# Siyou-Li/u2Tokenizer

Measured on AMD Instinct MI355X. Metric: CT volumes/sec (256^3 fp16) through u2Tokenizer fwd, higher is better.
Workload: dtype bf16; 1 GPU; BASELINE configs[2]: u2Qwen3-8B-shaped path, 256^3 volume = 8x(32,256,256) fp16, ViT-B 3D x12, SPP, 4-layer rma+diffts+dmtp tokenizer (8 heads, top_k 1024, scales {1,2,4}, 256 queries), text 1024, prompt 1024; hidden_size=4096, batch_per_gpu=1, streams_per_gpu=2, parallelism=replicas x1, tta_side_stream=off in the multi-stream run, on in the one-stream run

## Files before the change

include/u2tok.h:

```cpp
#ifndef U2TOK_H_
#define U2TOK_H_

#include <stddef.h>
#include <stdint.h>

#ifdef __cplusplus
extern "C" {
#endif

#define U2TOK_OK 0
#define U2TOK_ERR_ARG (-1)
#define U2TOK_ERR_LAUNCH (-2)
#define U2TOK_ERR_WORKSPACE (-3)
#define U2TOK_ERR_DEVICE (-4)

typedef void* u2tok_stream_t;

int u2tok_version(void);
const char* u2tok_arch(void);
const char* u2tok_elem(void);
int u2tok_device_check(void);
typedef struct u2tok_ctx* u2tok_ctx_t;
int u2tok_ctx_create(u2tok_ctx_t* out);
int u2tok_ctx_destroy(u2tok_ctx_t ctx);
// ... 67 lines not shown
int u2tok_tokenizer_forward(const u2tok_tokenizer_config* cfg, const void* const* weights, const void* v_token,
                            const void* t_token, void* out, int64_t* topk_idx_out, void* svr_out, void* workspace,
                            size_t workspace_bytes, u2tok_stream_t stream);

typedef struct {
  const void* const* svr_in;
  void* const* svr_out;
  const void* visual_in;
  void* visual_out;
  const void* const* tta_in;
  void* const* tta_out;
} u2tok_tokenizer_taps;
int u2tok_tokenizer_forward_taps(const u2tok_tokenizer_config* cfg, const void* const* weights, const void* v_token,
                                 const void* t_token, void* out, int64_t* topk_idx_out, const u2tok_tokenizer_taps* taps,
                                 void* workspace, size_t workspace_bytes, u2tok_stream_t stream);

int u2tok_embed_splice(const void* table, const int64_t* ids, const void* feats, void* out, int32_t B, int32_t S,
                       int32_t E, int32_t nfeat, int64_t vocab, u2tok_stream_t stream);

size_t u2tok_preprocess_workspace_bytes(int32_t D, int32_t H, int32_t W);
int u2tok_preprocess_volume(const float* vol, void* out, int32_t* info, int32_t D, int32_t H, int32_t W, int32_t target,
                            int32_t depth_pad, float lower_pct, float upper_pct, int32_t out_dtype, void* workspace,
                            size_t workspace_bytes, u2tok_stream_t stream);

typedef struct {
  int32_t rot90_k;
  int32_t flip[3];
  float scale_factor;
  float shift_offset;
} u2tok_augment;
// ... 158 lines not shown
```

u2tokenizer_amd/_lib.py:

```python
from __future__ import annotations

import ctypes as C
import os
import subprocess
import threading
from pathlib import Path

_PKG = Path(__file__).resolve().parent
_LIB = _PKG / "lib" / "libu2tok_hip.so"
_LIBS = {"bf16": _LIB, "f16": _PKG / "lib" / "libu2tok_hip_f16.so"}
_lock = threading.Lock()
_handles = {}


class LibraryNotBuilt(RuntimeError):
    pass


def lib_path() -> Path:
    return _LIB


def build(verbose: bool = False) -> Path:
    cmd = ["make", "-C", str(_PKG / "csrc"), "-j", str(os.cpu_count() or 4)]
# ... 55 lines not shown
    "u2tok_ctx_destroy": (_i32, [_vp]),
    "u2tok_ctx_set_current": (_i32, [_vp]),
    "u2tok_ctx_get_current": (_vp, []),
    "u2tok_set_option": (_i32, [C.c_char_p, _i32]),
    "u2tok_profile_collect": (_i32, [_vp, _vp, _vp, _i32]),
    "u2tok_profile_collect2": (_i32, [_vp, _vp, _vp, _vp, _i32]),
    "u2tok_set_gemm_scratch": (_i32, [_vp, _sz, _vp]),
    "u2tok_vit_workspace_bytes": (_sz, [C.POINTER(VitConfig)]),
    "u2tok_vit_forward": (_i32, [C.POINTER(VitConfig), C.POINTER(_vp), _vp, _vp, _vp, _sz, _vp]),
    "u2tok_spp_workspace_bytes": (_sz, [C.POINTER(SppConfig)]),
    "u2tok_spp_forward": (_i32, [C.POINTER(SppConfig), C.POINTER(_vp), _vp, _vp, _vp, _sz, _vp]),
    "u2tok_tokenizer_workspace_bytes": (_sz, [C.POINTER(TokConfig)]),
    "u2tok_tokenizer_forward": (_i32, [C.POINTER(TokConfig), C.POINTER(_vp), _vp, _vp, _vp, _vp, _vp, _vp, _sz, _vp]),
    "u2tok_tokenizer_forward_taps": (_i32, [C.POINTER(TokConfig), C.POINTER(_vp), _vp, _vp, _vp, _vp, C.POINTER(TokTaps),
                                            _vp, _sz, _vp]),
    "u2tok_tok_attention_workspace_bytes": (_sz, [_i32, _i32, _i32, _i32, _i32]),
    "u2tok_tok_attention": (_i32, [_vp, _vp, _vp, _vp, _i32, _i32, _i32, _i32, _i32, _i64, _i64, _i64, _i64, _i64, _i64, _i64,
                                   _i64, _f32, _vp, _i32, _i32, _vp, _sz, _vp]),
    "u2tok_preprocess_workspace_bytes": (_sz, [_i32, _i32, _i32]),
    "u2tok_preprocess_volume": (_i32, [_vp, _vp, _vp, _i32, _i32, _i32, _i32, _i32, _f32, _f32, _i32, _vp, _sz, _vp]),
    "u2tok_preprocess_volume_aug": (_i32, [_vp, _vp, _vp, _i32, _i32, _i32, _i32, _i32, _f32, _f32, _i32,
                                           C.POINTER(Augment), _vp, _sz, _vp]),
    "u2tok_embed_splice": (_i32, [_vp, _vp, _vp, _vp, _i32, _i32, _i32, _i32, _i64, _vp]),
    "u2tok_gemm_bf16": (_i32, [_vp, _vp, _vp, _vp, _vp, _i32, _i32, _i32, _i64, _i64, _i64, _i64, _i32, _i32,
                               _i64, _i64, _i64, _i64, _i64, _i64, _i64, _i64, _f32, _i32, _vp]),
    "u2tok_layernorm_bf16": (_i32, [_vp, _vp, _vp, _vp, _vp, _i32, _i32, _f32, _vp]),
    "u2tok_softmax_rows": (_i32, [_vp, _vp, _i32, _i32, _i32, _i64, _i64, _f32, _vp, _i32, _i32, _vp]),
    "u2tok_transpose_bf16": (_i32, [_vp, _vp, _i32, _i32, _i32, _i64, _i64, _i64, _i64, _i32, _vp]),
    "u2tok_im2col_patches": (_i32, [_vp, _i32, _vp, _i32, _i32, _i32, _i32, _i32, _i32, _i32, _vp]),
    "u2tok_avgpool3d_tokens": (_i32, [_vp, _vp, _i32, _i32, _i32, _i32, _i32, _i32, _i32, _i32, _vp]),
# ... 109 lines not shown
```

u2tokenizer_amd/csrc/capi.hip:

```cpp
#include <math.h>
#include <string.h>
#include <new>
#include "pipeline.h"

using namespace u2;

static_assert(U2TOK_OK == U2_OK && U2TOK_ERR_ARG == U2_ERR_ARG && U2TOK_ERR_LAUNCH == U2_ERR_LAUNCH &&
                  U2TOK_ERR_WORKSPACE == U2_ERR_WORKSPACE && U2TOK_ERR_DEVICE == U2_ERR_DEVICE,
              "public and internal status codes must agree");

#define BF(p) reinterpret_cast<const bf16_t*>(p)
#define BFW(p) reinterpret_cast<bf16_t*>(p)
#define ST(s) reinterpret_cast<hipStream_t>(s)

extern "C" {

int u2tok_version(void) { return 200;  }
const char* u2tok_arch(void) { return "gfx950"; }
const char* u2tok_elem(void) { return U2_ELEM_ASM; }

int u2tok_device_check(void) {
  int dev = 0;
  if (hipGetDevice(&dev) != hipSuccess) return U2_ERR_DEVICE;
  hipDeviceProp_t prop;
// ... 21 lines not shown

int u2tok_set_option(const char* name, int value) {
  if (!name) return U2_ERR_ARG;
  Options& o = ctx().opt;
  struct Opt { const char* name; int Options::*field; int lo, hi; };
  static const Opt table[] = {
      {"gemm_splitk", &Options::gemm_splitk, -1, 16},   {"gemm_mubuf", &Options::gemm_mubuf, 0, 1}, {"ln_wide", &Options::ln_wide, 0, 1},   {"gemm_big", &Options::gemm_big, -1, 27},
      {"gemm_big_grid", &Options::gemm_big_grid, 1, 4096}, {"gemm_big_splitk", &Options::gemm_big_splitk, 0, 16},
      {"gemm_big_drain", &Options::gemm_big_drain, 0, 1}, {"gemm_skinny", &Options::gemm_skinny, 0, 2},
       {"kmajor_b", &Options::kmajor_b, 0, 1},            {"gemm_tail_fused", &Options::gemm_tail_fused, 0, 1},
      {"flash_mode", &Options::flash_mode, 0, 7},        {"flash_q_prescaled", &Options::flash_q_prescaled, 0, 1},
      {"vit_flash", &Options::vit_flash, 0, 1},         {"tta_overlap", &Options::tta_overlap, 0, 1},
      {"vit_vt_epilogue", &Options::vit_vt_epilogue, 0, 1},
      {"tok_flash", &Options::tok_flash, 0, 1},
      {"tok_wide", &Options::tok_wide, 0, 2},
  };
  if (!strcmp(name, "gemm_tile")) {
    if (value != 0 && value != 64 && value != 128) return U2_ERR_ARG;
    o.gemm_tile = value;
    return U2_OK;
  }
  if (!strcmp(name, "profile")) { prof_enable(value != 0); return U2_OK; }
  for (const Opt& t : table)
    if (!strcmp(name, t.name)) {
      if (value < t.lo || value > t.hi) return U2_ERR_ARG;
      if (t.field == &Options::gemm_big && value > 0 && !(value >= 20 && value <= 27 && value != 23 && value != 25)) return U2_ERR_ARG;
      if (t.field == &Options::flash_mode && value != 0 && value != 1 && value != 7) return U2_ERR_ARG;
      o.*(t.field) = value;
      return U2_OK;
    }
// ... 29 lines not shown
size_t u2tok_spp_workspace_bytes(const u2tok_spp_config* cfg) {
  if (!cfg) return 0;
  size_t peak = 0;
  if (spp_forward(*cfg, nullptr, nullptr, nullptr, nullptr, 0, true, &peak, nullptr) != U2_OK) return 0;
  return peak + 256;
}
int u2tok_spp_forward(const u2tok_spp_config* cfg, const void* const* weights, const void* x, void* out,
                      void* workspace, size_t workspace_bytes, u2tok_stream_t stream) {
  if (!cfg || !workspace || ((uintptr_t)workspace & 255)) return U2_ERR_ARG;
  return spp_forward(*cfg, weights, BF(x), BFW(out), workspace, workspace_bytes, false, nullptr, ST(stream));
}

size_t u2tok_tokenizer_workspace_bytes(const u2tok_tokenizer_config* cfg) {
  if (!cfg) return 0;
  size_t peak = 0;
  if (tokenizer_forward(*cfg, nullptr, nullptr, nullptr, nullptr, nullptr, nullptr, nullptr, nullptr, 0, true, &peak,
                        nullptr) != U2_OK)
    return 0;
  return peak + 256;
}
int u2tok_tokenizer_forward(const u2tok_tokenizer_config* cfg, const void* const* weights, const void* v_token,
                            const void* t_token, void* out, int64_t* topk_idx_out, void* svr_out, void* workspace,
                            size_t workspace_bytes, u2tok_stream_t stream) {
  if (!cfg || !workspace || ((uintptr_t)workspace & 255)) return U2_ERR_ARG;
  return tokenizer_forward(*cfg, weights, BF(v_token), BF(t_token), BFW(out), topk_idx_out, BFW(svr_out), nullptr, workspace,
                           workspace_bytes, false, nullptr, ST(stream));
}
int u2tok_tokenizer_forward_taps(const u2tok_tokenizer_config* cfg, const void* const* weights, const void* v_token,
                                 const void* t_token, void* out, int64_t* topk_idx_out, const u2tok_tokenizer_taps* taps,
                                 void* workspace, size_t workspace_bytes, u2tok_stream_t stream) {
  if (!cfg || !taps || !workspace || ((uintptr_t)workspace & 255)) return U2_ERR_ARG;
  return tokenizer_forward(*cfg, weights, BF(v_token), BF(t_token), BFW(out), topk_idx_out, nullptr, taps, workspace,
                           workspace_bytes, false, nullptr, ST(stream));
}

size_t u2tok_preprocess_workspace_bytes(int32_t D, int32_t H, int32_t W) { return preprocess_workspace_bytes(D, H, W); }
int u2tok_preprocess_volume(const float* vol, void* out, int32_t* info, int32_t D, int32_t H, int32_t W, int32_t target,
                            int32_t depth_pad, float lower_pct, float upper_pct, int32_t out_dtype, void* workspace,
                            size_t workspace_bytes, u2tok_stream_t stream) {
  return preprocess_volume(vol, out, info, D, H, W, target, depth_pad, lower_pct, upper_pct, out_dtype, nullptr, workspace,
                           workspace_bytes, ST(stream));
}
int u2tok_preprocess_volume_aug(const float* vol, void* out, int32_t* info, int32_t D, int32_t H, int32_t W, int32_t target,
                                int32_t depth_pad, float lower_pct, float upper_pct, int32_t out_dtype,
                                const u2tok_augment* aug, void* workspace, size_t workspace_bytes, u2tok_stream_t stream) {
  if (!aug) return U2_ERR_ARG;
  PreAugment a;
  a.rot_k = aug->rot90_k;
// ... 324 lines not shown
```

u2tokenizer_amd/csrc/ctx.h:

```cpp
#pragma once
#include <mutex>
#include <vector>
#include "common.h"

namespace u2 {

struct Options {
  int ln_wide = 1;
  int gemm_tile = 0;
  int gemm_mubuf = 1;
  int gemm_splitk = 0;
  int gemm_big = 0;
  int gemm_big_grid = 256;
  int gemm_big_splitk = 0;
  int gemm_big_drain = 1;
  int gemm_skinny = 2;
  int gemm_tail_fused = 1;
  int kmajor_b = 1;
  int flash_mode = 0;
  int flash_q_prescaled = 0;
  int vit_flash = 1;
  int vit_vt_epilogue = 1;
  int tok_flash = 1;
  int tok_wide = 2;
  int tta_overlap = 1;
  int profile = 0;
};

struct SideStream {
  hipStream_t owner = nullptr;
  hipStream_t s = nullptr;
  hipEvent_t fork = nullptr;
  hipEvent_t done[16] = {};
};

struct Scratch {
  hipStream_t st;
  void* p;
  size_t bytes;
};
// ... 30 lines not shown
```

u2tokenizer_amd/csrc/pipeline.h:

```cpp
#pragma once
#include <algorithm>
#include "../../include/u2tok.h"
#include "kernels.h"

namespace u2 {

typedef u2tok_vit_config VitConfig;
typedef u2tok_spp_config SppConfig;
typedef u2tok_tokenizer_config TokConfig;
typedef u2tok_tokenizer_taps TokTaps;

int vit_forward(const VitConfig& c, const void* const* W, const void* volume, bf16_t* out, void* ws, size_t ws_bytes,
                bool dry, size_t* peak, hipStream_t st);
int spp_forward(const SppConfig& c, const void* const* W, const bf16_t* x, bf16_t* out, void* ws, size_t ws_bytes,
                bool dry, size_t* peak, hipStream_t st);
int tokenizer_forward(const TokConfig& c, const void* const* W, const bf16_t* v_token, const bf16_t* t_token,
                      bf16_t* out, int64_t* topk_idx_out, bf16_t* svr_out, const TokTaps* taps, void* ws, size_t ws_bytes,
                      bool dry, size_t* peak, hipStream_t st);

}
```

u2tokenizer_amd/csrc/pipeline.hip:

```cpp
#include "pipeline.h"

namespace u2 {

namespace {

struct Arena {
  char* base;
  size_t cap;
  size_t off = 0, peak = 0;
  bool dry;
  Arena(void* b, size_t c, bool d) : base((char*)b), cap(c), dry(d) {}
  template <typename T>
  T* get(size_t count) {
    const size_t a = (off + 255) & ~(size_t)255;
    off = a + count * sizeof(T);
    if (off > peak) peak = off;
    if (dry) return reinterpret_cast<T*>((uintptr_t)0x1000 + a);
    return (off <= cap) ? reinterpret_cast<T*>(base + a) : nullptr;
  }
  bool ok() const { return dry || peak <= cap; }
};

struct ScratchScope {
  Context& cx;
// ... 275 lines not shown
  return a.wk && a.bk && a.wv == a.wk + (size_t)E * E && a.bv == a.bk + E;
}
inline bool qkv_packed(const Att& a, int E) {
  return a.wq && a.bq && a.wk == a.wq + (size_t)E * E && a.bk == a.bq + E && kv_packed(a, E);
}
int qkv_proj(const bf16_t* x, const Att& a, bf16_t* out, int64_t rows, int E, bool dry, hipStream_t st) {
  if (!dry && qkv_packed(a, E)) {
    U2_RUN(linear(x, E, a.wq, a.bq, out, 3 * E, rows, E, 3 * E, 0, nullptr, 0, st));
    return U2_OK;
  }
  U2_RUN(linear(x, E, a.wq, a.bq, out, 3 * E, rows, E, E, 0, nullptr, 0, st));
  U2_RUN(linear(x, E, a.wk, a.bk, out + E, 3 * E, rows, E, E, 0, nullptr, 0, st));
  U2_RUN(linear(x, E, a.wv, a.bv, out + 2 * E, 3 * E, rows, E, E, 0, nullptr, 0, st));
  return U2_OK;
}
}

int tokenizer_forward(const TokConfig& c, const void* const* W, const bf16_t* v_token, const bf16_t* t_token,
                      bf16_t* out, int64_t* topk_idx_out, bf16_t* svr_out, const TokTaps* taps, void* ws, size_t ws_bytes,
                      bool dry, size_t* peak, hipStream_t st) {
  if (c.B <= 0 || c.T <= 0 || c.N <= 0 || c.E <= 0 || c.Lt <= 0 || c.num_heads <= 0 || c.num_layers < 0) return U2_ERR_ARG;
  if (c.E % c.num_heads || (c.E / c.num_heads) % 8 || c.top_k <= 0 || c.num_query <= 0) return U2_ERR_ARG;
  if (c.attn_type < 0 || c.attn_type > 2) return U2_ERR_ARG;
  if (!dry && (!W || !v_token || !t_token || !out)) return U2_ERR_ARG;
  const int B = c.B, T = c.T, N = c.N, E = c.E, H = c.num_heads, d = E / H, L = c.num_layers, Q = c.num_query;
  const int TN = T * N, k = c.top_k;
  if (!c.enable_diffts && k > TN) return U2_ERR_ARG;
  if (N > c.max_seq_len || T > c.max_seq_len || Q > c.max_seq_len) return U2_ERR_ARG;
  const float scale = 1.0f / sqrtf((float)d);
  auto wp = [&](int i) { return dry ? nullptr : reinterpret_cast<const bf16_t*>(W[i]); };
  auto att_at = [&](int i) {
    Att a{wp(i), wp(i + 1), wp(i + 2), wp(i + 3), wp(i + 4), wp(i + 5), wp(i + 6), wp(i + 7), wp(i + 8)};
    if (c.attn_type != 0) a.rb = nullptr;
    return a;
  };
  const int i_sel = 1 + 18 * L, i_gate = i_sel + 2, i_tta = i_gate + 2, i_lin = i_tta + 33 * L;

  Arena ar(ws, ws_bytes, dry);
  const size_t kSplitK = std::max<size_t>(24u << 20, (size_t)16 * B * c.num_query * 3 * E);
  char* skw = ar.get<char>(kSplitK);
  U2_CHECK_WS(ar);
  Context& cx = ctx();
  ScratchScope scratch_scope(cx, st, skw, kSplitK, !dry);
  const int64_t rows = (int64_t)B * TN;
  bf16_t* xa = ar.get<bf16_t>((size_t)rows * E);
  bf16_t* xb = ar.get<bf16_t>((size_t)rows * E);
  bf16_t* qkv = ar.get<bf16_t>((size_t)rows * 3 * E);
  bf16_t* ctx = ar.get<bf16_t>((size_t)rows * E);
  U2_CHECK_WS(ar);

  const bf16_t* x = v_token;
  for (int l = 0; l < L; ++l) {
    const Att sp = att_at(1 + 18 * l), tp = att_at(1 + 18 * l + 9);
    if (taps && !dry && taps->svr_in && taps->svr_in[l]) x = reinterpret_cast<const bf16_t*>(taps->svr_in[l]);
// ... 157 lines not shown
  if (overlap && !dry) {
    if (hipEventRecord(side->fork, st) != hipSuccess || hipStreamWaitEvent(side->s, side->fork, 0) != hipSuccess)
      return U2_ERR_LAUNCH;
    for (int l = 0; l < L; ++l) {
      const int base = i_tta + 33 * l;
      Att va = att_at(base + 9), ta = att_at(base + 18);
      { const int e = kv_proj(va, V, Lv, kv_v[l], side->s); if (e != U2_OK) return e; }
      if (hipEventRecord(side->done[2 * l], side->s) != hipSuccess) return U2_ERR_LAUNCH;
      { const int e = kv_proj(ta, t_token, c.Lt, kv_t[l], side->s); if (e != U2_OK) return e; }
      if (hipEventRecord(side->done[2 * l + 1], side->s) != hipSuccess) return U2_ERR_LAUNCH;
    }
    const Att la = att_at(i_lin);
    U2_RUN(linear(V, E, la.wk, la.bk, k_lin, E, (int64_t)B * Lv, E, E, 0, nullptr, 0, side->s));
    if (hipEventRecord(side->done[2 * L], side->s) != hipSuccess) return U2_ERR_LAUNCH;
  }
  U2_RUN(fill_rows(wp(0), qa, B, (int64_t)Q * E, (int64_t)Q * E, st));
  bf16_t* qcur = qa;
  auto cross = [&](const Att& a, const bf16_t* src, int Ls, const bf16_t* qin, bf16_t* dst, bf16_t* kv,
                   int kv_ready) -> int {
    U2_RUN(linear(qin, E, a.wq, a.bq, qproj, E, qrows, E, E, 0, nullptr, 0, st));
    if (kv_ready < 0) {
      const int e = kv_proj(a, src, Ls, kv, st);
      if (e != U2_OK) return e;
    } else if (!dry) {
      if (hipStreamWaitEvent(st, side->done[kv_ready], 0) != hipSuccess) return U2_ERR_LAUNCH;
    }
    AttnCore ac{qproj, kv, kv + E, E, 2 * E, 2 * E, (int64_t)Q * E, (int64_t)Ls * 2 * E, (int64_t)Ls * 2 * E,
                qctx, E, (int64_t)Q * E, B, Q, Ls, H, d, scale, nullptr, 0};
    const int e = attention_core(ar, ac, dry, st);
    if (e != U2_OK) return e;
    U2_RUN(linear(qctx, E, a.wd, a.bd, dst, E, qrows, E, E, 0, nullptr, 0, st));
    return U2_OK;
  };
  for (int l = 0; l < L; ++l) {
    const int base = i_tta + 33 * l;
    const Att sa = att_at(base);
    Att va = att_at(base + 9), ta = att_at(base + 18);
    va.rb = ta.rb = nullptr;
    const bf16_t *ns_w = wp(base + 27), *ns_b = wp(base + 28), *nv_w = wp(base + 29), *nv_b = wp(base + 30),
                 *nt_w = wp(base + 31), *nt_b = wp(base + 32);
    if (taps && !dry && taps->tta_in && taps->tta_in[l]) qcur = (bf16_t*)taps->tta_in[l];
    bf16_t* s1 = (qcur == qa) ? qb : qa;
    bf16_t* s2 = qc;
    if (c.attn_type == 2 && B == 1) {
      U2_RUN(linear(qcur, E, sa.wv, sa.bv, qctx, E, qrows, E, E, 0, nullptr, 0, st));
    } else if (c.attn_type == 2) {
      { const int e = qkv_proj(qcur, sa, qproj, qrows, E, dry, st); if (e != U2_OK) return e; }
      const int e = chunk_axis_attention(ar, qproj, qctx, 1, B, Q, H, d, scale, nullptr, c.max_seq_len, dry, st);
      if (e != U2_OK) return e;
    } else {
      { const int e = qkv_proj(qcur, sa, qproj, qrows, E, dry, st); if (e != U2_OK) return e; }
      if (c.attn_type == 1) {
        U2_RUN(rope_apply(qproj, B, Q, 1, H, d, 3 * E, c.max_seq_len, 0, st));
        U2_RUN(rope_apply(qproj + E, B, Q, 1, H, d, 3 * E, c.max_seq_len, 0, st));
      }
      AttnCore ac{qproj, qproj + E, qproj + 2 * E, 3 * E, 3 * E, 3 * E, (int64_t)Q * 3 * E, (int64_t)Q * 3 * E,
                  (int64_t)Q * 3 * E, qctx, E, (int64_t)Q * E, B, Q, Q, H, d, scale, sa.rb, c.max_seq_len};
      const int e = attention_core(ar, ac, dry, st);
      if (e != U2_OK) return e;
    }
    U2_RUN(linear(qctx, E, sa.wd, sa.bd, qo, E, qrows, E, E, 0, nullptr, 0, st));
    U2_RUN(layernorm_bf16(qcur, qo, ns_w, ns_b, s1, 1, (int)qrows, E, 0, E, 0, E, 0, E, c.ln_eps, st));
    { const int e = cross(va, V, Lv, s1, qo, overlap ? kv_v[l] : kv_inline, overlap ? 2 * l : -1); if (e != U2_OK) return e; }
    U2_RUN(layernorm_bf16(s1, qo, nv_w, nv_b, s2, 1, (int)qrows, E, 0, E, 0, E, 0, E, c.ln_eps, st));
    { const int e = cross(ta, t_token, c.Lt, s2, qo, overlap ? kv_t[l] : kv_inline, overlap ? 2 * l + 1 : -1); if (e != U2_OK) return e; }
    U2_RUN(layernorm_bf16(s2, qo, nt_w, nt_b, s1, 1, (int)qrows, E, 0, E, 0, E, 0, E, c.ln_eps, st));
    qcur = s1;
    if (taps && !dry && taps->tta_out && taps->tta_out[l] &&
        hipMemcpyAsync(taps->tta_out[l], qcur, (size_t)qrows * E * sizeof(bf16_t), hipMemcpyDeviceToDevice, st) != hipSuccess)
      return U2_ERR_LAUNCH;
  }
  {
    const Att la = att_at(i_lin);
    U2_RUN(linear(qcur, E, la.wq, la.bq, qproj, E, qrows, E, E, 0, nullptr, 0, st));
    if (!overlap) {
      U2_RUN(linear(V, E, la.wk, la.bk, k_lin, E, (int64_t)B * Lv, E, E, 0, nullptr, 0, st));
    } else if (!dry) {
      if (hipStreamWaitEvent(st, side->done[2 * L], 0) != hipSuccess) return U2_ERR_LAUNCH;
    }
    AttnCore ac{qproj, k_lin, V, E, E, E, (int64_t)Q * E, (int64_t)Lv * E, (int64_t)Lv * E,
                out, E, (int64_t)Q * E, B, Q, Lv, H, d, scale, nullptr, 0};
    const int e = attention_core(ar, ac, dry, st);
// ... 9 lines not shown
```

u2tokenizer_amd/ops.py:

```python
from __future__ import annotations

import contextlib
import ctypes as C
import functools
import threading
from typing import Optional

import torch

from . import _lib

GEMM_BIAS_N, GEMM_BIAS_M, GEMM_GELU, GEMM_RESIDUAL, GEMM_OUT_F32 = 1, 2, 4, 8, 16
_VOL_DTYPE = {torch.float16: 0, torch.bfloat16: 1, torch.float32: 2}


class Context:

    def __init__(self):
        self._handles = {}
        self._options = {}
        self._scratch = {}
        self._lock = threading.Lock()
        self.handle_for("bf16")

# ... 37 lines not shown

    def close(self) -> None:
        with self._lock:
            handles, self._handles = self._handles, {}
        for elem, hd in handles.items():
            _lib.load_library(elem).u2tok_ctx_destroy(hd)

    @staticmethod
    def _set(h, hd, name, value):
        prev = h.u2tok_ctx_get_current()
        h.u2tok_ctx_set_current(hd)
        try:
            _lib.check(h.u2tok_set_option(name.encode(), int(value)), f"u2tok_set_option({name})")
        finally:
            h.u2tok_ctx_set_current(prev)

    def set_option(self, name: str, value: int) -> None:
        with self._lock:
            self._options[name] = int(value)
            handles = list(self._handles.items())
        for elem, hd in handles:
            self._set(_lib.load_library(elem), hd, name, value)

    def __enter__(self):
        stack = getattr(_tls, "stack", None)
        if stack is None:
            stack = _tls.stack = []
        stack.append(self)
        return self

# ... 1015 lines not shown
```

u2tokenizer_amd/tokenizer.py:

```python
from __future__ import annotations

import ctypes as C

import torch
import torch.nn as nn

from . import _lib, ops

_ATTN_TYPES = {"rma": 0, "rope": 1}


def _init_attn(m):
    for lin in (m.wq, m.wk, m.wv, m.dense):
        nn.init.xavier_uniform_(lin.weight)
        if lin.bias is not None:
            nn.init.zeros_(lin.bias)


class RelativeMultiheadAttention(nn.Module):

    def __init__(self, d_model, num_heads, max_seq_len=512):
        super().__init__()
        assert d_model % num_heads == 0
        self.num_heads, self.d_model, self.depth, self.max_seq_len = num_heads, d_model, d_model // num_heads, max_seq_len
# ... 154 lines not shown
        return [m.wq.weight, m.wq.bias, m.wk.weight, m.wk.bias, None, None, None, None, None]
    if isinstance(m, nn.MultiheadAttention):
        E = m.embed_dim
        W, b = m.in_proj_weight, m.in_proj_bias
        return [W[:E], b[:E], W[E:2 * E], b[E:2 * E], W[2 * E:], b[2 * E:], m.out_proj.weight, m.out_proj.bias, None]
    return [m.wq.weight, m.wq.bias, m.wk.weight, m.wk.bias, m.wv.weight, m.wv.bias, m.dense.weight, m.dense.bias,
            getattr(m, "relative_bias", None)]


def _unshare_packed(module, state_dict, prefix, local_metadata):
    for k, v in list(state_dict.items()):
        if k.startswith(prefix) and torch.is_tensor(v) and \
                v.untyped_storage().nbytes() != v.numel() * v.element_size():
            state_dict[k] = v.detach().clone() if not v.requires_grad else v.clone().detach()
    return state_dict


class u2Tokenizer(nn.Module):

    def __init__(self, embed_size, num_heads, num_layers, top_k, use_multi_scale, num_3d_query_token, hidden_size,
                 attn_type="rma", enable_diffts=False, enable_dmtp=False):
        super().__init__()
        if embed_size != hidden_size:
            raise ValueError("embed_size must equal hidden_size (builder.py:5,11 pass config.hidden_size for both)")
        self.svt_module = SpatioTemporalVisualTokenRefinerModel(
            embed_size=embed_size, num_heads=num_heads, num_layers=num_layers, top_k=top_k,
            use_multi_scale=use_multi_scale, attn_type=attn_type, enable_diffts=enable_diffts,
            enable_dmtp=enable_dmtp)
        self.tta_module = TextConditionTokenAggregatorModel(d_model=embed_size, num_layers=num_layers,
                                                            num_heads=num_heads, attn_type=attn_type)
        self.query_tokens = nn.Parameter(torch.zeros(1, num_3d_query_token, hidden_size))
        self.query_tokens.data.normal_(mean=0.0, std=0.02)
        self.embed_size, self.num_heads, self.num_layers, self.top_k = embed_size, num_heads, num_layers, top_k
        self.use_multi_scale, self.num_query, self.attn_type = bool(use_multi_scale), num_3d_query_token, attn_type
        self.enable_diffts, self.enable_dmtp = bool(enable_diffts), bool(enable_dmtp)
        self._ws = ops._Workspace()
        self._packed_key = None
        self._dead_offloaded = False
        self._register_state_dict_hook(_unshare_packed)
        self.last_topk_indices = None
        self.capture_svr_tokens = False
        self.last_svr_tokens = None

    def _weights(self):
        w = [self.query_tokens]
        for layer in self.svt_module.attention_network.layers:
            w += _att_ptrs(layer.spatial_attention) + _att_ptrs(layer.temporal_attention)
        sn = self.svt_module.token_selection.score_net
        w += [sn.weight, sn.bias]
        if self.enable_dmtp:
            w += [self.svt_module.dynamic_pool.gate_fc.weight, self.svt_module.dynamic_pool.gate_fc.bias]
        else:
# ... 9 lines not shown
    def pack_weights(self) -> None:
        key = (self.query_tokens.data_ptr(), self.query_tokens.dtype)
        if self._packed_key == key:
            return
        with torch.no_grad():
            for layer in self.svt_module.attention_network.layers:
                _pack_qkv(layer.spatial_attention)
                _pack_qkv(layer.temporal_attention)
            for layer in self.tta_module.layers_vt:
                for m in (layer.self_attention, layer.visual_cross_attention, layer.text_cross_attention):
                    _pack_qkv(m)
        if self.query_tokens.is_cuda:
            torch.cuda.synchronize(self.query_tokens.device)
        self._packed_key = key

    def _apply(self, fn, *args, **kwargs):
        r = super()._apply(fn, *args, **kwargs)
        self._packed_key = None
        if self.query_tokens.is_cuda:
            self.pack_weights()
            if self._dead_offloaded:
                self.offload_dead_parameters()
        return r

    def dead_parameters(self):
        la = self.tta_module.layer_linagg.linear_aggregator
        return [la.wv.weight, la.wv.bias, la.dense.weight, la.dense.bias]

    def offload_dead_parameters(self) -> int:
        freed = 0
        for p in self.dead_parameters():
            if p.is_cuda:
                freed += p.numel() * p.element_size()
# ... 45 lines not shown
            return arr

        svr_out = [torch.empty((B, T, N, E), dtype=ops.elem_dtype(), device=dev) for _ in range(L)]
        tta_out = [torch.empty((B, Q, E), dtype=ops.elem_dtype(), device=dev) for _ in range(L)]
        visual_out = torch.empty((B, Lv, E), dtype=ops.elem_dtype(), device=dev)
        if visual_in is not None:
            visual_in = ops._need(visual_in, ops.ELEM, "visual_in").contiguous()
            assert tuple(visual_in.shape) == (B, Lv, E)
        taps = _lib.TokTaps(svr_in=ptr_array(svr_in, (B, T, N, E)), svr_out=ptr_array(svr_out, (B, T, N, E)),
                            visual_in=None if visual_in is None else visual_in.data_ptr(), visual_out=visual_out.data_ptr(),
                            tta_in=ptr_array(tta_in, (B, Q, E)), tta_out=ptr_array(tta_out, (B, Q, E)))
        with ops.on_device(v_token) as (h, stream):
            ws = self._ws.get(nbytes, dev)
            out = torch.empty((B, Q, E), dtype=ops.elem_dtype(), device=dev)
            idx = None if self.enable_diffts else torch.empty((B, self.top_k), dtype=torch.int64, device=dev)
            _lib.check(h.u2tok_tokenizer_forward_taps(C.byref(cfg), table, v_token.data_ptr(), t_token.data_ptr(),
                                                      out.data_ptr(), None if idx is None else idx.data_ptr(),
                                                      C.byref(taps), ws.data_ptr(), ws.numel(), stream),
                       "u2tok_tokenizer_forward_taps")
        self.last_topk_indices = idx
        return out, {"svr_out": svr_out, "visual_out": visual_out, "tta_out": tta_out}

    def _config(self, B, T, N, E, Lt):
        return _lib.TokConfig(B=B, T=T, N=N, E=E, Lt=Lt, num_heads=self.num_heads,
                              num_layers=self.num_layers, top_k=self.top_k, num_query=self.num_query,
                              use_multi_scale=int(self.use_multi_scale), attn_type=_ATTN_TYPES.get(self.attn_type, 2),
                              enable_diffts=int(self.enable_diffts), enable_dmtp=int(self.enable_dmtp),
                              max_seq_len=512, diffts_tau=float(getattr(self.svt_module.token_selection, "tau", 1.0)),
                              ln_eps=1e-5)

    def forward(self, v_token, t_token):
        with ops.on_device(v_token, elem=self.query_tokens.dtype):
            return self._forward(v_token, t_token)

# ... 18 lines not shown
        self._check_envelope(B, T, N, E, t_token.shape[1])
        cfg = self._config(B, T, N, E, t_token.shape[1])
        table = ops.weight_table(self._weights())
        nbytes = h.u2tok_tokenizer_workspace_bytes(C.byref(cfg))
        if nbytes == 0:
            raise RuntimeError("u2tok_tokenizer_workspace_bytes rejected the configuration "
                               f"(B={B}, T={T}, N={N}, E={E}, heads={self.num_heads}, top_k={self.top_k})")
        idx = svr = None
        with ops.on_device(v_token) as (h, stream):
            ws = self._ws.get(nbytes, v_token.device)
            out = torch.empty((B, self.num_query, E), dtype=ops.elem_dtype(), device=v_token.device)
            if not self.enable_diffts:
                idx = torch.empty((B, self.top_k), dtype=torch.int64, device=v_token.device)
            if self.capture_svr_tokens:
                svr = torch.empty((B, T * N, E), dtype=ops.elem_dtype(), device=v_token.device)
            _lib.check(h.u2tok_tokenizer_forward(C.byref(cfg), table, v_token.data_ptr(), t_token.data_ptr(),
                                                 out.data_ptr(), None if idx is None else idx.data_ptr(),
                                                 None if svr is None else svr.data_ptr(), ws.data_ptr(), ws.numel(),
                                                 stream), "u2tok_tokenizer_forward")
        self.last_topk_indices = idx
        self.last_svr_tokens = svr
        return out
```

Baseline: 127.7 volumes/s.

## Precompute and cache input-independent TTA layer-0 query prefix across calls

The first TTA layer's self-attention block and visual-cross query projection depend only on learned query tokens and weights. This change computes them once into a cached buffer keyed on parameter pointers, versions and options, and reuses it in every forward call. That removes a query self-attention, layernorm and a linear per call. Because the cached values are a pure function of the weights, the result stays correct when weights change, at the cost of extra key-checking logic and a synchronize on recompute.

Result: no change. 127.2 volumes/s (-0.4%).

```diff
diff --git a/include/u2tok.h b/include/u2tok.h
--- a/include/u2tok.h
+++ b/include/u2tok.h
@@ -105,6 +105,16 @@
 int u2tok_tokenizer_forward_taps(const u2tok_tokenizer_config* cfg, const void* const* weights, const void* v_token,
                                  const void* t_token, void* out, int64_t* topk_idx_out, const u2tok_tokenizer_taps* taps,
                                  void* workspace, size_t workspace_bytes, u2tok_stream_t stream);
+
+size_t u2tok_tokenizer_tta_prefix_bytes(const u2tok_tokenizer_config* cfg);
+int u2tok_tokenizer_tta_prefix(const u2tok_tokenizer_config* cfg, const void* const* weights, void* prefix_out, void* workspace,
+                               size_t workspace_bytes, u2tok_stream_t stream);
+int u2tok_tokenizer_forward_ex(const u2tok_tokenizer_config* cfg, const void* const* weights, const void* v_token,
+                               const void* t_token, void* out, int64_t* topk_idx_out, void* svr_out, const void* tta_prefix,
+                               void* workspace, size_t workspace_bytes, u2tok_stream_t stream);
+int u2tok_tokenizer_forward_taps_ex(const u2tok_tokenizer_config* cfg, const void* const* weights, const void* v_token,
+                                    const void* t_token, void* out, int64_t* topk_idx_out, const u2tok_tokenizer_taps* taps,
+                                    const void* tta_prefix, void* workspace, size_t workspace_bytes, u2tok_stream_t stream);
 
 int u2tok_embed_splice(const void* table, const int64_t* ids, const void* feats, void* out, int32_t B, int32_t S,
                        int32_t E, int32_t nfeat, int64_t vocab, u2tok_stream_t stream);
diff --git a/u2tokenizer_amd/_lib.py b/u2tokenizer_amd/_lib.py
--- a/u2tokenizer_amd/_lib.py
+++ b/u2tokenizer_amd/_lib.py
@@ -93,6 +93,11 @@
     "u2tok_tokenizer_forward": (_i32, [C.POINTER(TokConfig), C.POINTER(_vp), _vp, _vp, _vp, _vp, _vp, _vp, _sz, _vp]),
     "u2tok_tokenizer_forward_taps": (_i32, [C.POINTER(TokConfig), C.POINTER(_vp), _vp, _vp, _vp, _vp, C.POINTER(TokTaps),
                                             _vp, _sz, _vp]),
+    "u2tok_tokenizer_tta_prefix_bytes": (_sz, [C.POINTER(TokConfig)]),
+    "u2tok_tokenizer_tta_prefix": (_i32, [C.POINTER(TokConfig), C.POINTER(_vp), _vp, _vp, _sz, _vp]),
+    "u2tok_tokenizer_forward_ex": (_i32, [C.POINTER(TokConfig), C.POINTER(_vp), _vp, _vp, _vp, _vp, _vp, _vp, _vp, _sz, _vp]),
+    "u2tok_tokenizer_forward_taps_ex": (_i32, [C.POINTER(TokConfig), C.POINTER(_vp), _vp, _vp, _vp, _vp, C.POINTER(TokTaps),
+                                               _vp, _vp, _sz, _vp]),
     "u2tok_tok_attention_workspace_bytes": (_sz, [_i32, _i32, _i32, _i32, _i32]),
     "u2tok_tok_attention": (_i32, [_vp, _vp, _vp, _vp, _i32, _i32, _i32, _i32, _i32, _i64, _i64, _i64, _i64, _i64, _i64, _i64,
                                    _i64, _f32, _vp, _i32, _i32, _vp, _sz, _vp]),
diff --git a/u2tokenizer_amd/csrc/capi.hip b/u2tokenizer_amd/csrc/capi.hip
--- a/u2tokenizer_amd/csrc/capi.hip
+++ b/u2tokenizer_amd/csrc/capi.hip
@@ -59,6 +59,7 @@
       {"vit_vt_epilogue", &Options::vit_vt_epilogue, 0, 1},
       {"tok_flash", &Options::tok_flash, 0, 1},
       {"tok_wide", &Options::tok_wide, 0, 2},
+      {"tta_prefix", &Options::tta_prefix, 0, 1},
   };
   if (!strcmp(name, "gemm_tile")) {
     if (value != 0 && value != 64 && value != 128) return U2_ERR_ARG;
@@ -118,24 +119,42 @@
 size_t u2tok_tokenizer_workspace_bytes(const u2tok_tokenizer_config* cfg) {
   if (!cfg) return 0;
   size_t peak = 0;
-  if (tokenizer_forward(*cfg, nullptr, nullptr, nullptr, nullptr, nullptr, nullptr, nullptr, nullptr, 0, true, &peak,
+  if (tokenizer_forward(*cfg, nullptr, nullptr, nullptr, nullptr, nullptr, nullptr, nullptr, nullptr, nullptr, 0, true, &peak,
                         nullptr) != U2_OK)
     return 0;
   return peak + 256;
 }
+int u2tok_tokenizer_forward_ex(const u2tok_tokenizer_config* cfg, const void* const* weights, const void* v_token,
+                               const void* t_token, void* out, int64_t* topk_idx_out, void* svr_out, const void* tta_prefix,
+                               void* workspace, size_t workspace_bytes, u2tok_stream_t stream) {
+  if (!cfg || !workspace || ((uintptr_t)workspace & 255) || ((uintptr_t)tta_prefix & 255)) return U2_ERR_ARG;
+  return tokenizer_forward(*cfg, weights, BF(v_token), BF(t_token), BFW(out), topk_idx_out, BFW(svr_out), nullptr, BF(tta_prefix),
+                           workspace, workspace_bytes, false, nullptr, ST(stream));
+}
 int u2tok_tokenizer_forward(const u2tok_tokenizer_config* cfg, const void* const* weights, const void* v_token,
                             const void* t_token, void* out, int64_t* topk_idx_out, void* svr_out, void* workspace,
                             size_t workspace_bytes, u2tok_stream_t stream) {
-  if (!cfg || !workspace || ((uintptr_t)workspace & 255)) return U2_ERR_ARG;
-  return tokenizer_forward(*cfg, weights, BF(v_token), BF(t_token), BFW(out), topk_idx_out, BFW(svr_out), nullptr, workspace,
-                           workspace_bytes, false, nullptr, ST(stream));
+  return u2tok_tokenizer_forward_ex(cfg, weights, v_token, t_token, out, topk_idx_out, svr_out, nullptr, workspace,
+                                    workspace_bytes, stream);
+}
+int u2tok_tokenizer_forward_taps_ex(const u2tok_tokenizer_config* cfg, const void* const* weights, const void* v_token,
+                                    const void* t_token, void* out, int64_t* topk_idx_out, const u2tok_tokenizer_taps* taps,
+                                    const void* tta_prefix, void* workspace, size_t workspace_bytes, u2tok_stream_t stream) {
+  if (!cfg || !taps || !workspace || ((uintptr_t)workspace & 255) || ((uintptr_t)tta_prefix & 255)) return U2_ERR_ARG;
+  return tokenizer_forward(*cfg, weights, BF(v_token), BF(t_token), BFW(out), topk_idx_out, nullptr, taps, BF(tta_prefix),
+                           workspace, workspace_bytes, false, nullptr, ST(stream));
 }
 int u2tok_tokenizer_forward_taps(const u2tok_tokenizer_config* cfg, const void* const* weights, const void* v_token,
                                  const void* t_token, void* out, int64_t* topk_idx_out, const u2tok_tokenizer_taps* taps,
                                  void* workspace, size_t workspace_bytes, u2tok_stream_t stream) {
-  if (!cfg || !taps || !workspace || ((uintptr_t)workspace & 255)) return U2_ERR_ARG;
-  return tokenizer_forward(*cfg, weights, BF(v_token), BF(t_token), BFW(out), topk_idx_out, nullptr, taps, workspace,
-                           workspace_bytes, false, nullptr, ST(stream));
+  return u2tok_tokenizer_forward_taps_ex(cfg, weights, v_token, t_token, out, topk_idx_out, taps, nullptr, workspace,
+                                         workspace_bytes, stream);
+}
+size_t u2tok_tokenizer_tta_prefix_bytes(const u2tok_tokenizer_config* cfg) { return cfg ? tokenizer_tta_prefix_bytes(*cfg) : 0; }
+int u2tok_tokenizer_tta_prefix(const u2tok_tokenizer_config* cfg, const void* const* weights, void* prefix_out, void* workspace,
+                               size_t workspace_bytes, u2tok_stream_t stream) {
+  if (!cfg || !prefix_out || ((uintptr_t)prefix_out & 255) || !workspace || ((uintptr_t)workspace & 255)) return U2_ERR_ARG;
+  return tokenizer_tta_prefix(*cfg, weights, BFW(prefix_out), workspace, workspace_bytes, false, nullptr, ST(stream));
 }
 
 size_t u2tok_preprocess_workspace_bytes(int32_t D, int32_t H, int32_t W) { return preprocess_workspace_bytes(D, H, W); }
diff --git a/u2tokenizer_amd/csrc/ctx.h b/u2tokenizer_amd/csrc/ctx.h
--- a/u2tokenizer_amd/csrc/ctx.h
+++ b/u2tokenizer_amd/csrc/ctx.h
@@ -24,6 +24,7 @@
   int tok_flash = 1;
   int tok_wide = 2;
   int tta_overlap = 1;
+  int tta_prefix = 1;
   int profile = 0;
 };
 
diff --git a/u2tokenizer_amd/csrc/pipeline.h b/u2tokenizer_amd/csrc/pipeline.h
--- a/u2tokenizer_amd/csrc/pipeline.h
+++ b/u2tokenizer_amd/csrc/pipeline.h
@@ -15,7 +15,10 @@
 int spp_forward(const SppConfig& c, const void* const* W, const bf16_t* x, bf16_t* out, void* ws, size_t ws_bytes,
                 bool dry, size_t* peak, hipStream_t st);
 int tokenizer_forward(const TokConfig& c, const void* const* W, const bf16_t* v_token, const bf16_t* t_token,
-                      bf16_t* out, int64_t* topk_idx_out, bf16_t* svr_out, const TokTaps* taps, void* ws, size_t ws_bytes,
-                      bool dry, size_t* peak, hipStream_t st);
+                      bf16_t* out, int64_t* topk_idx_out, bf16_t* svr_out, const TokTaps* taps, const bf16_t* tta_prefix,
+                      void* ws, size_t ws_bytes, bool dry, size_t* peak, hipStream_t st);
+size_t tokenizer_tta_prefix_bytes(const TokConfig& c);
+int tokenizer_tta_prefix(const TokConfig& c, const void* const* W, bf16_t* prefix_out, void* ws, size_t ws_bytes, bool dry,
+                         size_t* peak, hipStream_t st);
 
 }
diff --git a/u2tokenizer_amd/csrc/pipeline.hip b/u2tokenizer_amd/csrc/pipeline.hip
--- a/u2tokenizer_amd/csrc/pipeline.hip
+++ b/u2tokenizer_amd/csrc/pipeline.hip
@@ -313,30 +313,125 @@
   U2_RUN(linear(x, E, a.wv, a.bv, out + 2 * E, 3 * E, rows, E, E, 0, nullptr, 0, st));
   return U2_OK;
 }
-}
-
-int tokenizer_forward(const TokConfig& c, const void* const* W, const bf16_t* v_token, const bf16_t* t_token,
-                      bf16_t* out, int64_t* topk_idx_out, bf16_t* svr_out, const TokTaps* taps, void* ws, size_t ws_bytes,
-                      bool dry, size_t* peak, hipStream_t st) {
+
+int tok_check_config(const TokConfig& c) {
   if (c.B <= 0 || c.T <= 0 || c.N <= 0 || c.E <= 0 || c.Lt <= 0 || c.num_heads <= 0 || c.num_layers < 0) return U2_ERR_ARG;
   if (c.E % c.num_heads || (c.E / c.num_heads) % 8 || c.top_k <= 0 || c.num_query <= 0) return U2_ERR_ARG;
   if (c.attn_type < 0 || c.attn_type > 2) return U2_ERR_ARG;
+  if (!c.enable_diffts && c.top_k > c.T * c.N) return U2_ERR_ARG;
+  if (c.N > c.max_seq_len || c.T > c.max_seq_len || c.num_query > c.max_seq_len) return U2_ERR_ARG;
+  return U2_OK;
+}
+inline const bf16_t* tok_w(const void* const* W, int i, bool dry) { return dry ? nullptr : reinterpret_cast<const bf16_t*>(W[i]); }
+inline Att tok_att(const TokConfig& c, const void* const* W, int i, bool dry) {
+  Att a{tok_w(W, i, dry),     tok_w(W, i + 1, dry), tok_w(W, i + 2, dry), tok_w(W, i + 3, dry), tok_w(W, i + 4, dry),
+        tok_w(W, i + 5, dry), tok_w(W, i + 6, dry), tok_w(W, i + 7, dry), tok_w(W, i + 8, dry)};
+  if (c.attn_type != 0) a.rb = nullptr;
+  return a;
+}
+inline int tok_tta_base(const TokConfig& c) { return 1 + 18 * c.num_layers + 4; }
+inline size_t tok_splitk_bytes(const TokConfig& c) {
+  return std::max<size_t>(24u << 20, (size_t)16 * c.B * c.num_query * 3 * c.E);
+}
+
+struct TtaScratch {
+  Arena& ar;
+  bf16_t *qproj, *qctx, *qo;
+  bool dry;
+  hipStream_t st;
+};
+
+int tta_self_block(const TokConfig& c, const TtaScratch& t, const Att& sa, const bf16_t* ns_w, const bf16_t* ns_b,
+                   const bf16_t* qcur, bf16_t* s1) {
+  const int B = c.B, E = c.E, H = c.num_heads, d = E / H, Q = c.num_query;
+  const int64_t qrows = (int64_t)B * Q;
+  const float scale = 1.0f / sqrtf((float)d);
+  const bool dry = t.dry;
+  hipStream_t st = t.st;
+  bf16_t *qproj = t.qproj, *qctx = t.qctx, *qo = t.qo;
+  if (c.attn_type == 2 && B == 1) {
+    U2_RUN(linear(qcur, E, sa.wv, sa.bv, qctx, E, qrows, E, E, 0, nullptr, 0, st));
+  } else if (c.attn_type == 2) {
+    { const int e = qkv_proj(qcur, sa, qproj, qrows, E, dry, st); if (e != U2_OK) return e; }
+    const int e = chunk_axis_attention(t.ar, qproj, qctx, 1, B, Q, H, d, scale, nullptr, c.max_seq_len, dry, st);
+    if (e != U2_OK) return e;
+  } else {
+    { const int e = qkv_proj(qcur, sa, qproj, qrows, E, dry, st); if (e != U2_OK) return e; }
+    if (c.attn_type == 1) {
+      U2_RUN(rope_apply(qproj, B, Q, 1, H, d, 3 * E, c.max_seq_len, 0, st));
+      U2_RUN(rope_apply(qproj + E, B, Q, 1, H, d, 3 * E, c.max_seq_len, 0, st));
+    }
+    AttnCore ac{qproj, qproj + E, qproj + 2 * E, 3 * E, 3 * E, 3 * E, (int64_t)Q * 3 * E, (int64_t)Q * 3 * E,
+                (int64_t)Q * 3 * E, qctx, E, (int64_t)Q * E, B, Q, Q, H, d, scale, sa.rb, c.max_seq_len};
+    const int e = attention_core(t.ar, ac, dry, st);
+    if (e != U2_OK) return e;
+  }
+  U2_RUN(linear(qctx, E, sa.wd, sa.bd, qo, E, qrows, E, E, 0, nullptr, 0, st));
+  U2_RUN(layernorm_bf16(qcur, qo, ns_w, ns_b, s1, 1, (int)qrows, E, 0, E, 0, E, 0, E, c.ln_eps, st));
+  return U2_OK;
+}
+
+int tta_query_prefix(const TokConfig& c, const void* const* W, const TtaScratch& t, bf16_t* qa, bf16_t* s1, bf16_t* qproj0) {
+  const int E = c.E, Q = c.num_query, base = tok_tta_base(c);
+  const int64_t qrows = (int64_t)c.B * Q;
+  const bool dry = t.dry;
+  hipStream_t st = t.st;
+  U2_RUN(fill_rows(tok_w(W, 0, dry), qa, c.B, (int64_t)Q * E, (int64_t)Q * E, st));
+  const int e = tta_self_block(c, t, tok_att(c, W, base, dry), tok_w(W, base + 27, dry), tok_w(W, base + 28, dry), qa, s1);
+  if (e != U2_OK) return e;
+  const Att va = tok_att(c, W, base + 9, dry);
+  U2_RUN(linear(s1, E, va.wq, va.bq, qproj0, E, qrows, E, E, 0, nullptr, 0, st));
+  return U2_OK;
+}
+inline size_t tta_prefix_half_bytes(const TokConfig& c) {
+  return (size_t)round_up((int64_t)c.B * c.num_query * c.E * (int64_t)sizeof(bf16_t), 256);
+}
+}
+
+size_t tokenizer_tta_prefix_bytes(const TokConfig& c) {
+  if (tok_check_config(c) != U2_OK || c.num_layers <= 0) return 0;
+  return 2 * tta_prefix_half_bytes(c);
+}
+
+int tokenizer_tta_prefix(const TokConfig& c, const void* const* W, bf16_t* prefix_out, void* ws, size_t ws_bytes, bool dry,
+                         size_t* peak, hipStream_t st) {
+  { const int e = tok_check_config(c); if (e != U2_OK) return e; }
+  if (c.num_layers <= 0) return U2_ERR_ARG;
+  if (!dry && (!W || !prefix_out)) return U2_ERR_ARG;
+  const int64_t qrows = (int64_t)c.B * c.num_query;
+  const int E = c.E;
+  Arena ar(ws, ws_bytes, dry);
+  const size_t kSplitK = tok_splitk_bytes(c);
+  char* skw = ar.get<char>(kSplitK);
+  U2_CHECK_WS(ar);
+  ScratchScope scratch_scope(ctx(), st, skw, kSplitK, !dry);
+  bf16_t* qa = ar.get<bf16_t>((size_t)qrows * E);
+  TtaScratch t{ar, ar.get<bf16_t>((size_t)qrows * 3 * E), ar.get<bf16_t>((size_t)qrows * E), ar.get<bf16_t>((size_t)qrows * E),
+               dry, st};
+  U2_CHECK_WS(ar);
+  bf16_t* s1 = prefix_out;
+  bf16_t* qproj0 = dry ? nullptr : reinterpret_cast<bf16_t*>(reinterpret_cast<char*>(prefix_out) + tta_prefix_half_bytes(c));
+  const int e = tta_query_prefix(c, W, t, qa, s1, qproj0);
+  if (e != U2_OK) return e;
+  if (peak) *peak = ar.peak;
+  U2_CHECK_WS(ar);
+  return U2_OK;
+}
+
+int tokenizer_forward(const TokConfig& c, const void* const* W, const bf16_t* v_token, const bf16_t* t_token,
+                      bf16_t* out, int64_t* topk_idx_out, bf16_t* svr_out, const TokTaps* taps, const bf16_t* tta_prefix,
+                      void* ws, size_t ws_bytes, bool dry, size_t* peak, hipStream_t st) {
+  { const int e = tok_check_config(c); if (e != U2_OK) return e; }
   if (!dry && (!W || !v_token || !t_token || !out)) return U2_ERR_ARG;
   const int B = c.B, T = c.T, N = c.N, E = c.E, H = c.num_heads, d = E / H, L = c.num_layers, Q = c.num_query;
   const int TN = T * N, k = c.top_k;
-  if (!c.enable_diffts && k > TN) return U2_ERR_ARG;
-  if (N > c.max_seq_len || T > c.max_seq_len || Q > c.max_seq_len) return U2_ERR_ARG;
   const float scale = 1.0f / sqrtf((float)d);
-  auto wp = [&](int i) { return dry ? nullptr : reinterpret_cast<const bf16_t*>(W[i]); };
-  auto att_at = [&](int i) {
-    Att a{wp(i), wp(i + 1), wp(i + 2), wp(i + 3), wp(i + 4), wp(i + 5), wp(i + 6), wp(i + 7), wp(i + 8)};
-    if (c.attn_type != 0) a.rb = nullptr;
-    return a;
-  };
-  const int i_sel = 1 + 18 * L, i_gate = i_sel + 2, i_tta = i_gate + 2, i_lin = i_tta + 33 * L;
+  auto wp = [&](int i) { return tok_w(W, i, dry); };
+  auto att_at = [&](int i) { return tok_att(c, W, i, dry); };
+  const int i_sel = 1 + 18 * L, i_gate = i_sel + 2, i_tta = tok_tta_base(c), i_lin = i_tta + 33 * L;
 
   Arena ar(ws, ws_bytes, dry);
-  const size_t kSplitK = std::max<size_t>(24u << 20, (size_t)16 * B * c.num_query * 3 * E);
+  const size_t kSplitK = tok_splitk_bytes(c);
   char* skw = ar.get<char>(kSplitK);
   U2_CHECK_WS(ar);
   Context& cx = ctx();
@@ -524,18 +619,28 @@
     U2_RUN(linear(V, E, la.wk, la.bk, k_lin, E, (int64_t)B * Lv, E, E, 0, nullptr, 0, side->s));
     if (hipEventRecord(side->done[2 * L], side->s) != hipSuccess) return U2_ERR_LAUNCH;
   }
-  U2_RUN(fill_rows(wp(0), qa, B, (int64_t)Q * E, (int64_t)Q * E, st));
-  bf16_t* qcur = qa;
-  auto cross = [&](const Att& a, const bf16_t* src, int Ls, const bf16_t* qin, bf16_t* dst, bf16_t* kv,
+  const bool l0_forced = taps && !dry && taps->tta_in && taps->tta_in[0];
+  const bool l0_head = L > 0 && !l0_forced;
+  const bool use_prefix = !dry && l0_head && tta_prefix && opts().tta_prefix;
+  const bf16_t* pre_s1 = use_prefix ? tta_prefix : nullptr;
+  const bf16_t* pre_q = use_prefix ? reinterpret_cast<const bf16_t*>(reinterpret_cast<const char*>(tta_prefix) + tta_prefix_half_bytes(c))
+                                   : nullptr;
+  const TtaScratch tsc{ar, qproj, qctx, qo, dry, st};
+  if (!l0_head) U2_RUN(fill_rows(wp(0), qa, B, (int64_t)Q * E, (int64_t)Q * E, st));
+  const bf16_t* qcur = qa;
+  auto cross = [&](const Att& a, const bf16_t* src, int Ls, const bf16_t* qin, const bf16_t* qp, bf16_t* dst, bf16_t* kv,
                    int kv_ready) -> int {
-    U2_RUN(linear(qin, E, a.wq, a.bq, qproj, E, qrows, E, E, 0, nullptr, 0, st));
+    if (!qp) {
+      U2_RUN(linear(qin, E, a.wq, a.bq, qproj, E, qrows, E, E, 0, nullptr, 0, st));
+      qp = qproj;
+    }
     if (kv_ready < 0) {
       const int e = kv_proj(a, src, Ls, kv, st);
       if (e != U2_OK) return e;
     } else if (!dry) {
       if (hipStreamWaitEvent(st, side->done[kv_ready], 0) != hipSuccess) return U2_ERR_LAUNCH;
     }
-    AttnCore ac{qproj, kv, kv + E, E, 2 * E, 2 * E, (int64_t)Q * E, (int64_t)Ls * 2 * E, (int64_t)Ls * 2 * E,
+    AttnCore ac{qp, kv, kv + E, E, 2 * E, 2 * E, (int64_t)Q * E, (int64_t)Ls * 2 * E, (int64_t)Ls * 2 * E,
                 qctx, E, (int64_t)Q * E, B, Q, Ls, H, d, scale, nullptr, 0};
     const int e = attention_core(ar, ac, dry, st);
     if (e != U2_OK) return e;
@@ -549,33 +654,27 @@
     va.rb = ta.rb = nullptr;
     const bf16_t *ns_w = wp(base + 27), *ns_b = wp(base + 28), *nv_w = wp(base + 29), *nv_b = wp(base + 30),
                  *nt_w = wp(base + 31), *nt_b = wp(base + 32);
-    if (taps && !dry && taps->tta_in && taps->tta_in[l]) qcur = (bf16_t*)taps->tta_in[l];
-    bf16_t* s1 = (qcur == qa) ? qb : qa;
+    if (taps && !dry && taps->tta_in && taps->tta_in[l]) qcur = reinterpret_cast<const bf16_t*>(taps->tta_in[l]);
+    bf16_t* s3 = (qcur == qa) ? qb : qa;
+    const bf16_t* s1 = s3;
     bf16_t* s2 = qc;
-    if (c.attn_type == 2 && B == 1) {
-      U2_RUN(linear(qcur, E, sa.wv, sa.bv, qctx, E, qrows, E, E, 0, nullptr, 0, st));
-    } else if (c.attn_type == 2) {
-      { const int e = qkv_proj(qcur, sa, qproj, qrows, E, dry, st); if (e != U2_OK) return e; }
-      const int e = chunk_axis_attention(ar, qproj, qctx, 1, B, Q, H, d, scale, nullptr, c.max_seq_len, dry, st);
+    const bf16_t* q0 = nullptr;
+    if (l == 0 && use_prefix) {
+      s1 = pre_s1;
+      q0 = pre_q;
+    } else if (l == 0 && l0_head) {
+      const int e = tta_query_prefix(c, W, tsc, qa, s3, qproj);
       if (e != U2_OK) return e;
+      q0 = qproj;
     } else {
-      { const int e = qkv_proj(qcur, sa, qproj, qrows, E, dry, st); if (e != U2_OK) return e; }
-      if (c.attn_type == 1) {
-        U2_RUN(rope_apply(qproj, B, Q, 1, H, d, 3 * E, c.max_seq_len, 0, st));
-        U2_RUN(rope_apply(qproj + E, B, Q, 1, H, d, 3 * E, c.max_seq_len, 0, st));
-      }
-      AttnCore ac{qproj, qproj + E, qproj + 2 * E, 3 * E, 3 * E, 3 * E, (int64_t)Q * 3 * E, (int64_t)Q * 3 * E,
-                  (int64_t)Q * 3 * E, qctx, E, (int64_t)Q * E, B, Q, Q, H, d, scale, sa.rb, c.max_seq_len};
-      const int e = attention_core(ar, ac, dry, st);
+      const int e = tta_self_block(c, tsc, sa, ns_w, ns_b, qcur, s3);
       if (e != U2_OK) return e;
     }
-    U2_RUN(linear(qctx, E, sa.wd, sa.bd, qo, E, qrows, E, E, 0, nullptr, 0, st));
-    U2_RUN(layernorm_bf16(qcur, qo, ns_w, ns_b, s1, 1, (int)qrows, E, 0, E, 0, E, 0, E, c.ln_eps, st));
-    { const int e = cross(va, V, Lv, s1, qo, overlap ? kv_v[l] : kv_inline, overlap ? 2 * l : -1); if (e != U2_OK) return e; }
+    { const int e = cross(va, V, Lv, s1, q0, qo, overlap ? kv_v[l] : kv_inline, overlap ? 2 * l : -1); if (e != U2_OK) return e; }
     U2_RUN(layernorm_bf16(s1, qo, nv_w, nv_b, s2, 1, (int)qrows, E, 0, E, 0, E, 0, E, c.ln_eps, st));
-    { const int e = cross(ta, t_token, c.Lt, s2, qo, overlap ? kv_t[l] : kv_inline, overlap ? 2 * l + 1 : -1); if (e != U2_OK) return e; }
-    U2_RUN(layernorm_bf16(s2, qo, nt_w, nt_b, s1, 1, (int)qrows, E, 0, E, 0, E, 0, E, c.ln_eps, st));
-    qcur = s1;
+    { const int e = cross(ta, t_token, c.Lt, s2, nullptr, qo, overlap ? kv_t[l] : kv_inline, overlap ? 2 * l + 1 : -1); if (e != U2_OK) return e; }
+    U2_RUN(layernorm_bf16(s2, qo, nt_w, nt_b, s3, 1, (int)qrows, E, 0, E, 0, E, 0, E, c.ln_eps, st));
+    qcur = s3;
     if (taps && !dry && taps->tta_out && taps->tta_out[l] &&
         hipMemcpyAsync(taps->tta_out[l], qcur, (size_t)qrows * E * sizeof(bf16_t), hipMemcpyDeviceToDevice, st) != hipSuccess)
       return U2_ERR_LAUNCH;
diff --git a/u2tokenizer_amd/ops.py b/u2tokenizer_amd/ops.py
--- a/u2tokenizer_amd/ops.py
+++ b/u2tokenizer_amd/ops.py
@@ -75,6 +75,10 @@
             _lib.check(h.u2tok_set_option(name.encode(), int(value)), f"u2tok_set_option({name})")
         finally:
             h.u2tok_ctx_set_current(prev)
+
+    def options_snapshot(self, skip=()) -> tuple:
+        with self._lock:
+            return tuple(sorted((k, v) for k, v in self._options.items() if k not in skip))
 
     def set_option(self, name: str, value: int) -> None:
         with self._lock:
diff --git a/u2tokenizer_amd/tokenizer.py b/u2tokenizer_amd/tokenizer.py
--- a/u2tokenizer_amd/tokenizer.py
+++ b/u2tokenizer_amd/tokenizer.py
@@ -1,6 +1,7 @@
 from __future__ import annotations
 
 import ctypes as C
+import threading
 
 import torch
 import torch.nn as nn
@@ -192,6 +193,14 @@
                 v.untyped_storage().nbytes() != v.numel() * v.element_size():
             state_dict[k] = v.detach().clone() if not v.requires_grad else v.clone().detach()
     return state_dict
+
+
+_PREFIX_NEUTRAL_OPTIONS = ("profile", "tta_prefix", "tta_overlap")
+_PREFIX_LOCK = threading.Lock()
+
+
+def tta_prefix_key(params, B, dtype, attn_type, options=()):
+    return (int(B), dtype, attn_type, tuple(options), tuple((p.data_ptr(), p._version) for p in params))
 
 
 class u2Tokenizer(nn.Module):
@@ -214,6 +223,8 @@
         self.enable_diffts, self.enable_dmtp = bool(enable_diffts), bool(enable_dmtp)
         self._ws = ops._Workspace()
         self._packed_key = None
+        self._prefix = None
+        self.prefix_recomputes = 0
         self._dead_offloaded = False
         self._register_state_dict_hook(_unshare_packed)
         self.last_topk_indices = None
@@ -253,9 +264,48 @@
             torch.cuda.synchronize(self.query_tokens.device)
         self._packed_key = key
 
+    def _prefix_params(self):
+        layer = self.tta_module.layers_vt[0]
+        sa, vq = layer.self_attention, layer.visual_cross_attention.wq
+        if isinstance(sa, nn.MultiheadAttention):
+            ps = [sa.in_proj_weight, sa.in_proj_bias, sa.out_proj.weight, sa.out_proj.bias]
+        else:
+            ps = [sa.wq.weight, sa.wq.bias, sa.wk.weight, sa.wk.bias, sa.wv.weight, sa.wv.bias, sa.dense.weight, sa.dense.bias]
+            if getattr(sa, "relative_bias", None) is not None:
+                ps.append(sa.relative_bias)
+        return [self.query_tokens] + ps + [layer.norm_self.weight, layer.norm_self.bias, vq.weight, vq.bias]
+
+    def invalidate_prefix(self) -> None:
+        self._prefix = None
+
+    def _tta_prefix(self, h, cfg, table, nbytes, device, stream):
+        if self.num_layers == 0:
+            return None
+        key = tta_prefix_key(self._prefix_params(), cfg.B, self.query_tokens.dtype, self.attn_type,
+                             ops.active_context(device).options_snapshot(skip=_PREFIX_NEUTRAL_OPTIONS))
+        ent = self._prefix
+        if ent is not None and ent[0] == key:
+            return ent[1]
+        with _PREFIX_LOCK:
+            ent = self._prefix
+            if ent is not None and ent[0] == key:
+                return ent[1]
+            pbytes = h.u2tok_tokenizer_tta_prefix_bytes(C.byref(cfg))
+            if pbytes == 0:
+                raise RuntimeError("u2tok_tokenizer_tta_prefix_bytes rejected the configuration")
+            buf = torch.empty(pbytes, dtype=torch.uint8, device=device)
+            ws = self._ws.get(nbytes, device)
+            _lib.check(h.u2tok_tokenizer_tta_prefix(C.byref(cfg), table, buf.data_ptr(), ws.data_ptr(), ws.numel(), stream),
+                       "u2tok_tokenizer_tta_prefix")
+            torch.cuda.synchronize(device)
+            self._prefix = (key, buf)
+            self.prefix_recomputes += 1
+            return buf
+
     def _apply(self, fn, *args, **kwargs):
         r = super()._apply(fn, *args, **kwargs)
         self._packed_key = None
+        self._prefix = None
         if self.query_tokens.is_cuda:
             self.pack_weights()
             if self._dead_offloaded:
@@ -331,10 +381,12 @@
             ws = self._ws.get(nbytes, dev)
             out = torch.empty((B, Q, E), dtype=ops.elem_dtype(), device=dev)
             idx = None if self.enable_diffts else torch.empty((B, self.top_k), dtype=torch.int64, device=dev)
-            _lib.check(h.u2tok_tokenizer_forward_taps(C.byref(cfg), table, v_token.data_ptr(), t_token.data_ptr(),
-                                                      out.data_ptr(), None if idx is None else idx.data_ptr(),
-                                                      C.byref(taps), ws.data_ptr(), ws.numel(), stream),
-                       "u2tok_tokenizer_forward_taps")
+            prefix = self._tta_prefix(h, cfg, table, nbytes, dev, stream)
+            _lib.check(h.u2tok_tokenizer_forward_taps_ex(C.byref(cfg), table, v_token.data_ptr(), t_token.data_ptr(),
+                                                         out.data_ptr(), None if idx is None else idx.data_ptr(),
+                                                         C.byref(taps), None if prefix is None else prefix.data_ptr(),
+                                                         ws.data_ptr(), ws.numel(), stream),
+                       "u2tok_tokenizer_forward_taps_ex")
         self.last_topk_indices = idx
         return out, {"svr_out": svr_out, "visual_out": visual_out, "tta_out": tta_out}
 
@@ -383,10 +435,12 @@
                 idx = torch.empty((B, self.top_k), dtype=torch.int64, device=v_token.device)
             if self.capture_svr_tokens:
                 svr = torch.empty((B, T * N, E), dtype=ops.elem_dtype(), device=v_token.device)
-            _lib.check(h.u2tok_tokenizer_forward(C.byref(cfg), table, v_token.data_ptr(), t_token.data_ptr(),
-                                                 out.data_ptr(), None if idx is None else idx.data_ptr(),
-                                                 None if svr is None else svr.data_ptr(), ws.data_ptr(), ws.numel(),
-                                                 stream), "u2tok_tokenizer_forward")
+            prefix = self._tta_prefix(h, cfg, table, nbytes, v_token.device, stream)
+            _lib.check(h.u2tok_tokenizer_forward_ex(C.byref(cfg), table, v_token.data_ptr(), t_token.data_ptr(),
+                                                    out.data_ptr(), None if idx is None else idx.data_ptr(),
+                                                    None if svr is None else svr.data_ptr(),
+                                                    None if prefix is None else prefix.data_ptr(), ws.data_ptr(), ws.numel(),
+                                                    stream), "u2tok_tokenizer_forward_ex")
         self.last_topk_indices = idx
         self.last_svr_tokens = svr
         return out
```
